# cloudflare/zkp-ecdsa

Hardware: AMD Instinct MI355X
Metric: proveSignatureList proofs/sec (higher is better)
Workload: dtype u32 (9x30-bit limbs, 256/258-bit modular integers); 1 GPU; B=65536 proofs/GPU/step, ring=65536 keys (n=16), per-key tables, secLevel=80, P-256+Tom-256, 24-bit combs, chunk=22016 x 3 lanes; parallelism=single GPU

## Files before the change

zkp-ecdsa_amd/csrc/engine.h:

```cpp
#pragma once
#include <hip/hip_runtime.h>
#include <stdint.h>
#include <atomic>
#include <cstdlib>
#include "../../include/zkattest.h"
#include "curve.h"
#include "rng.h"

struct Soa {
    uint32_t* p;
    uint32_t stride;
};
struct Soa3 {
    Soa x, y, z;
};
template <class M, int K = 2>
ZK_DEV Fe<M, K> soa_ld(const Soa& a, uint32_t e) {
    Fe<M, K> r;
#pragma unroll
    for (int l = 0; l < NLIMB; l++) r.l[l] = a.p[(size_t)l * a.stride + e];
    return r;
}
template <class M, int K>
ZK_DEV void soa_st(const Soa& a, uint32_t e, const Fe<M, K>& v) {
// ... 174 lines not shown
    uint32_t* t1_cnt;
    uint8_t* vbytes;
    uint32_t* vc;
    uint8_t* ph_msg;
    uint32_t* ph_wk;
    uint8_t* ph_nblk;
    TomList vd;
    Soa gk_f, gk_g;
    uint32_t* gk_swap;
    Soa gk_total;
    uint32_t* gk_csub;
    VTerms slot_terms, gk_terms, misc_terms;
    uint8_t* slot_class;
    uint32_t* slot_perm;
    uint32_t* slot_cnt;
    Soa4 slot_acc, gk_acc, misc_acc;
    Soa4 wide_acc;
    Soa sSg, sSh, sSkx, sSky, sSR, sSH, sSL;
    Soa pSR, pSH, pSL;
    Soa pa_x, pa_y, pa_sc;
    uint32_t* pa_tab;
    uint8_t* pa_dig;
    Soa3 pacc;
    Soa clx, cly;
    uint32_t* cl_tab;
    uint8_t* cl_dig;
    uint32_t* p256_ok;
};
void launch_offsets_monotonic(hipStream_t s, const uint64_t* d_off, uint64_t B, uint32_t* d_bad );
void launch_v_unpack(hipStream_t s, uint32_t sec, uint32_t count, const uint8_t* packed, const uint64_t* poff, uint64_t first, uint64_t base, uint8_t* out, uint64_t* uoff);
void launch_v_header_validate(hipStream_t s, const VWork& V, uint32_t count, const uint8_t* proofs, const uint64_t* off, uint64_t first);
void launch_v_front_r(hipStream_t s, const Workspace& W, const VWork& V, uint32_t count, const uint8_t* proofs, const uint64_t* off, uint64_t first);
void launch_v_front_q(hipStream_t s, const DevParams& P, const Workspace& W, const VWork& V, uint32_t count, const uint8_t* proofs, const uint64_t* off, const uint8_t* msg, uint64_t first);
void launch_v_challenges(hipStream_t s, const VWork& V, uint32_t count, const uint8_t* proofs, const uint64_t* off, const uint8_t* msg, uint64_t first, uint32_t parts);
void launch_v_exp_challenge_small(hipStream_t s, const Workspace& W, const VWork& V, uint32_t count, const uint8_t* proofs, const uint64_t* off, uint64_t first);
void launch_v_sample(hipStream_t s, const VWork& V, uint32_t count, const uint8_t* vseeds, uint64_t first);
void launch_v_sample_check(hipStream_t s, const VWork& V, uint32_t count);
void launch_v_exp_status(hipStream_t s, const Workspace& W, const VWork& V, uint32_t count, bool have_jm);
#define V_PH_MAXP 64
#define V_PH_BLOCKS 10
void launch_sha_msgs(hipStream_t s, const Workspace& W, uint32_t count, uint32_t* chal, uint32_t nblk, uint32_t ostride, const uint8_t* nblk_of = nullptr);
void launch_exph_hash(hipStream_t s, const Workspace& W, uint32_t count, uint32_t* chal);
void launch_v_exp_points(hipStream_t s, const Workspace& W, const VWork& V, uint32_t count, const uint8_t* proofs, const uint64_t* off, uint64_t first, uint32_t split = 1);
void launch_v_t1_scalars(hipStream_t s, const Workspace& W, const VWork& V, uint32_t count, const uint8_t* proofs, const uint64_t* off, uint64_t first);
void launch_v_derived(hipStream_t s, const Workspace& W, const VWork& V, uint32_t count, const uint8_t* proofs, const uint64_t* off, uint64_t first);
void launch_v_padd_hash(hipStream_t s, const DevParams& P, const Workspace& W, const VWork& V, uint32_t count, const uint8_t* proofs, const uint64_t* off, uint64_t first);
void launch_v_gk_total(hipStream_t s, const VWork& V, const Soa& ring, const uint32_t* etab, const int8_t* kdig, uint32_t count, uint32_t N, const uint8_t* proofs, const uint64_t* off, uint64_t first, const Soa& res, const Soa& res2);
#define GKM_MINN 12
size_t gkm_ring_frag_bytes(uint64_t N);
size_t gkm_coef_frag_bytes(uint32_t C);
void launch_gkm_ring_digits(hipStream_t s, const Soa& ring, uint32_t nblocks, int8_t* frag);
void launch_gkm_ring_digits_list(hipStream_t s, const Soa& ring, const uint32_t* d_blocks, uint32_t nb, int8_t* frag);
void launch_v_gk_block_mfma(hipStream_t s, const VWork& V, const int8_t* ring_frag, uint32_t nblocks, uint32_t count, int8_t* coef_frag, const Soa& res);
struct ChunkIn;
size_t gkm_etab_frag_bytes(uint64_t N);
size_t gkm_asub_frag_bytes(uint32_t C);
void launch_gkm_etab_digits(hipStream_t s, const uint32_t* E, uint32_t nblocks, int8_t* edig);
void launch_gkm_etab_digits_list(hipStream_t s, const uint32_t* E, uint32_t nblocks, const uint32_t* d_blocks, uint32_t nb, int8_t* edig);
void launch_gk_block_mfma(hipStream_t s, const Workspace& W, const ChunkIn& in, uint32_t nblocks, const Soa& res);
void launch_v_slot_points(hipStream_t s, const VWork& V, uint32_t count, const uint8_t* proofs, const uint64_t* off, uint64_t first);
void launch_v_slot_terms(hipStream_t s, const Workspace& W, const VWork& V, uint32_t count, const uint8_t* proofs, const uint64_t* off, const uint8_t* vseeds, uint64_t first);
void launch_v_proof_points(hipStream_t s, const VWork& V, uint32_t count, const uint8_t* proofs, const uint64_t* off, uint64_t first, uint32_t which);
void launch_v_proof_terms(hipStream_t s, const Workspace& W, const VWork& V, uint32_t count, const uint8_t* proofs, const uint64_t* off, const uint8_t* vseeds, uint64_t first);
void launch_v_proof_sums(hipStream_t s, const Workspace& W, const VWork& V, uint32_t count);
void launch_v_straus(hipStream_t s, const VTerms& L, uint32_t ngroups, uint32_t ng_stride, uint32_t n256, uint32_t n128, const Soa4& out,
                     const uint32_t* perm, const uint32_t* cnt, uint32_t tsplit = 1, uint32_t ostride = 1, uint32_t ny = 1, uint32_t ystride = 0);
void launch_v_acc_tree(hipStream_t s, const Soa4& src, uint32_t nouter, uint32_t width, const Soa4& dst, uint32_t dstride, uint32_t fill);
#ifndef ZK_COOP_MAX_CHAINS
#define ZK_COOP_MAX_CHAINS 16384u
#endif
#ifndef ZK_SCREEN_CO_MAX
#define ZK_SCREEN_CO_MAX 4096u
#endif
extern std::atomic<uint64_t> g_coop_chains;
static inline bool zk_one_lane_chains() {
    static const bool v = getenv("ZKATTEST_ONE_LANE_CHAINS") != nullptr;
    return v;
}
void launch_v_straus_co(hipStream_t s, const VTerms& L, uint32_t ngroups, uint32_t ng_stride, uint32_t n256, uint32_t n128, const Soa4& out, const uint32_t* perm,
                        const uint32_t* cnt, uint32_t tsplit, uint32_t ostride, uint32_t ny, uint32_t ystride);
void launch_v_p256_straus_co(hipStream_t s, const VWork& V, uint32_t count);
void launch_v_exp_points_co(hipStream_t s, const Workspace& W, const VWork& V, uint32_t count, const uint8_t* proofs, const uint64_t* off, uint64_t first);
void launch_rtab_base_co(hipStream_t s, const Workspace& W, uint32_t count, uint32_t bits, const uint8_t* skip);
void launch_v_slot_perm(hipStream_t s, const uint8_t* slot_class, uint32_t nslots, uint32_t* perm, uint32_t* cnt);
void launch_v_p256_straus(hipStream_t s, const VWork& V, uint32_t count, uint32_t per);
void launch_v_p256_total(hipStream_t s, const DevParams& P, const Workspace& W, const VWork& V, uint32_t count, uint32_t per);
void launch_v_p256_total_fixed(hipStream_t s, const DevParams& P, const Workspace& W, const VWork& V, uint32_t count);
void launch_v_p256_total_sum(hipStream_t s, const DevParams& P, const Workspace& W, const VWork& V, uint32_t count);
void launch_v_final(hipStream_t s, const Workspace& W, const VWork& V, uint32_t count, uint8_t* ok, int32_t* status, uint64_t first, const VGroupFlags& gf, uint32_t gsz);
void launch_v_final_memb(hipStream_t s, const Workspace& W, const VWork& V, uint32_t count, uint8_t* ok, int32_t* status, uint64_t first);
void launch_lv_census(hipStream_t s, uint64_t B, const uint8_t* proofs, const uint64_t* off, bool packed, uint8_t* cls, uint32_t* blk_cnt, uint32_t* out);
void launch_lv_perm(hipStream_t s, uint64_t B, const uint8_t* cls, const uint32_t* blk_base, const uint32_t* out, uint32_t* perm);
void launch_lv_gather_meta(hipStream_t s, uint32_t n, const uint32_t* sel, const uint64_t* off, const uint8_t* msg, const uint8_t* vseeds, uint64_t* w_off, uint8_t* w_msg,
                           uint8_t* w_seeds);
void launch_lv_gather_bytes(hipStream_t s, uint32_t n, const uint32_t* sel, const uint64_t* off, const uint8_t* proofs, const uint64_t* w_off, uint8_t* w_bytes);
void launch_lv_scatter(hipStream_t s, uint32_t n, const uint32_t* sel, const uint8_t* w_ok, const int32_t* w_st, uint8_t* ok, int32_t* status, int32_t st);
#define LV_BLOCK 1024
#define RG_UNKNOWN (ZK_MAX_RINGS * ZK_LV_CLASSES)
#define RG_CLASSES (RG_UNKNOWN + 1)
struct RingSlots {
    uint32_t id[ZK_MAX_RINGS];
    uint32_t count;
};
void launch_rg_census(hipStream_t s, uint64_t B, const uint32_t* ring_ids, const RingSlots& rs, const uint8_t* proofs, const uint64_t* off, bool packed, bool per_proof,
                      uint16_t* cls, uint32_t* blk_cnt, uint32_t* out);
void launch_rg_perm(hipStream_t s, uint64_t B, const uint16_t* cls, const uint32_t* blk_base, const uint32_t* out, uint32_t* perm);
// ... 334 lines not shown
```

zkp-ecdsa_amd/csrc/k_gk.hip:

```cpp
#include "engine.h"

#define GKB_BITS 8
#define GKB_SIZE 256

struct GkRankTab {
    uint8_t subset[256];
    uint8_t rank[256];
    uint16_t kstart[10];
};
constexpr GkRankTab gk_make_rank_tab() {
    GkRankTab t{};
    int r = 0;
    for (int k = 0; k <= 8; k++) {
        t.kstart[k] = (uint16_t)r;
        for (int s = 0; s < 256; s++) {
            int pc = 0;
            for (int b = 0; b < 8; b++) pc += (s >> b) & 1;
            if (pc == 8 - k) t.subset[r] = (uint8_t)s, t.rank[s] = (uint8_t)r, r++;
        }
    }
    t.kstart[9] = (uint16_t)r;
    return t;
}
__device__ const GkRankTab GK_RT = gk_make_rank_tab();

__global__ void __launch_bounds__(256) k_gk_etab(Soa ring, uint32_t nblocks, const uint32_t* __restrict__ blist, uint32_t nb, uint32_t* E) {
    uint64_t t = (uint64_t)blockIdx.x * blockDim.x + threadIdx.x;
    uint64_t total = (uint64_t)GKB_SIZE * GKB_SIZE * nb;
    if (t >= total) return;
    uint32_t block = (uint32_t)(t % nb);
    if (blist) block = blist[block];
    uint32_t lr = (uint32_t)(t / nb);
    uint32_t rank = lr & 255, llow = lr >> 8;
    uint32_t S = GK_RT.subset[rank];
    uint32_t fixed = llow & ~S;
    uint32_t pcS = __popc(S);
    Fe<ModQ, 1> acc = fe_zero<ModQ>();
    for (uint32_t T = S;; T = (T - 1) & S) {
        Fe<ModQ, 1> v = soa_ld<ModQ, 1>(ring, block * GKB_SIZE + (fixed | T));
        bool neg = (pcS - __popc(T)) & 1;
        acc = neg ? fe_sub_mod(acc, v) : fe_add_mod(acc, v);
        if (T == 0) break;
    }
    uint32_t o[9];
    limbs_repack<30, 29, 9, 9>(o, acc.l);
#pragma unroll
    for (int l = 0; l < 9; l++) E[((size_t)lr * 9 + l) * nblocks + block] = o[l];
}
void launch_gk_etab_list(hipStream_t s, const Soa& ring, uint32_t nblocks, const uint32_t* d_blocks, uint32_t nb, uint32_t* E) {
    uint64_t total = (uint64_t)GKB_SIZE * GKB_SIZE * nb;
    if (!total) return;
    hipLaunchKernelGGL(k_gk_etab, dim3((uint32_t)((total + 255) / 256)), dim3(256), 0, s, ring, nblocks, d_blocks, nb, E);
}
void launch_gk_etab(hipStream_t s, const Soa& ring, uint32_t nblocks, uint32_t* E) { launch_gk_etab_list(s, ring, nblocks, nullptr, nblocks, E); }
size_t gk_etab_words(uint64_t N) { return (size_t)GKB_SIZE * GKB_SIZE * 9 * (N / GKB_SIZE); }

// ... 39 lines not shown
ZK_DEV void gkc_zero(GkCols& a) {
#pragma unroll
    for (int i = 0; i < 18; i++) a.c[i] = 0;
}
ZK_DEV void gkc_carry(GkCols& a) {
#pragma unroll
    for (int i = 0; i < 17; i++) {
        a.c[i + 1] += a.c[i] >> 29;
        a.c[i] &= (1u << 29) - 1;
    }
}
ZK_DEV void gkc_mac(GkCols& a, const uint32_t x[9], const uint32_t y[9]) {
#pragma unroll
    for (int i = 0; i < 9; i++)
#pragma unroll
        for (int j = 0; j < 9; j++) a.c[i + j] = mad64(x[i], y[j], a.c[i + j]);
}
template <bool UNI>
__global__ void __launch_bounds__(256) k_gk_block(Workspace W, ChunkIn in, const uint32_t* __restrict__ E, const uint32_t* __restrict__ asub,
                                                  const uint32_t* __restrict__ order, const uint32_t* __restrict__ goff, uint32_t nblocks, uint32_t nwg, Soa res,
                                                  uint32_t kmask) {
    uint32_t w = blockIdx.x, seg = (nwg + 7) / 8;
    uint32_t widx = (w & 7) * seg + (w >> 3);
    if (widx >= nwg) return;
    uint32_t p, block;
    if (UNI) {
        uint32_t nbg = nblocks >> 8;
        uint32_t lo = 0, hi = GKB_SIZE;
        while (hi - lo > 1) {
            uint32_t mid = (lo + hi) >> 1;
            if (goff[mid] * nbg <= widx) lo = mid;
            else hi = mid;
        }
        uint32_t g0 = goff[lo], cnt = goff[lo + 1] - g0;
        uint32_t r = widx - g0 * nbg;
        p = order[g0 + r % cnt];
        block = (r / cnt) * 256 + threadIdx.x;
    } else {
        uint32_t slot = widx * 256 + threadIdx.x;
        if (slot >= in.count * nblocks) return;
        p = order[slot / nblocks];
        block = slot % nblocks;
    }
    uint32_t which = in.which[p];
    uint32_t llow = which & 255;
    const uint32_t* a = asub + (size_t)p * GKB_SIZE * 9;
    const uint32_t* e = E + (size_t)llow * GKB_SIZE * 9 * nblocks + block;
#pragma unroll 1
    for (uint32_t k = 0; k < 8; k++) {
        if (!((kmask >> k) & 1)) continue;
        GkCols acc;
        gkc_zero(acc);
        uint32_t r0 = GK_RT.kstart[k], r1 = GK_RT.kstart[k + 1];
#pragma unroll 1
        for (uint32_t rb = r0; rb < r1; rb += 7) {
            uint32_t re = rb + 7 < r1 ? rb + 7 : r1;
#pragma unroll 1
            for (uint32_t r = rb; r < re; r++) {
                uint32_t x[9], y[9];
#pragma unroll
                for (int l = 0; l < 9; l++) x[l] = a[r * 9 + l], y[l] = e[((size_t)r * 9 + l) * nblocks];
                gkc_mac(acc, x, y);
            }
            gkc_carry(acc);
        }
        uint32_t t29[18], t30[18];
#pragma unroll
        for (int i = 0; i < 18; i++) t29[i] = (uint32_t)acc.c[i];
        limbs_repack<29, 30, 18, 18>(t30, t29);
        Fe<ModQ, 1> c = fe_canon(redc_wide(t30));
        soa_st(res, (k * W.C + p) * nblocks + block, c);
    }
    soa_st(res, (8 * W.C + p) * nblocks + block, soa_ld<ModQ, 1>(W.ring, block * GKB_SIZE + llow));
}
void launch_gk_block_stage(hipStream_t s, const Workspace& W, const ChunkIn& in, const Soa& am, const Soa& res) {
    uint32_t nblocks = W.N >> GKB_BITS;
    const bool mm = W.gk_edig != nullptr && W.n >= GKM_MINN;
    hipLaunchKernelGGL(k_gk_sort, dim3(1), dim3(320), 0, s, in, W.gk_order, W.gk_goff, mm ? W.gk_toff : nullptr);
    hipLaunchKernelGGL(k_gk_asub, dim3(in.count), dim3(256), 0, s, W, in.count, am, W.gk_asub);
    bool uni = (nblocks & 255) == 0;
    uint32_t nwg = uni ? in.count * (nblocks >> 8) : (uint32_t)(((uint64_t)in.count * nblocks + 255) / 256);
    uint32_t grid = ((nwg + 7) / 8) * 8;
    const uint32_t kmask = mm ? 0x83u : 0xffu;
    if (uni) hipLaunchKernelGGL(k_gk_block<true>, dim3(grid), dim3(256), 0, s, W, in, W.gk_etab, W.gk_asub, W.gk_order, W.gk_goff, nblocks, nwg, res, kmask);
    else hipLaunchKernelGGL(k_gk_block<false>, dim3(grid), dim3(256), 0, s, W, in, W.gk_etab, W.gk_asub, W.gk_order, W.gk_goff, nblocks, nwg, res, kmask);
    if (mm) launch_gk_block_mfma(s, W, in, nblocks, res);
}

__global__ void __launch_bounds__(256) k_v_gk_csub(VWork V, uint32_t count, uint32_t* csub) {
    uint32_t t = gtid();
    if (t >= count * GKB_SIZE) return;
    uint32_t p = t >> 8, i = t & 255;
    Fe<ModQ, 2> acc = fe_one_mont<ModQ>().as<2>();
    bool zero = false;
    for (uint32_t j = 0; j < GKB_BITS; j++) {
        bool swap = V.gk_swap[j * V.C + p] != 0, set = (i >> j) & 1;
        if (swap) zero = zero || !set;
        else if (set) acc = acc * soa_ld<ModQ, 2>(V.gk_f, j * V.C + p);
    }
    Fe<ModQ, 1> c = zero ? fe_zero<ModQ>() : fe_canon(acc);
    uint32_t o[9];
    limbs_repack<30, 29, 9, 9>(o, c.l);
#pragma unroll
    for (int l = 0; l < 9; l++) csub[(size_t)t * 9 + l] = o[l];
}
template <bool UNI>
__global__ void __launch_bounds__(256) k_v_gk_block(uint32_t count, const uint32_t* __restrict__ E, const uint32_t* __restrict__ csub, uint32_t nblocks, Soa res) {
    uint32_t p, block;
    if (UNI) {
        uint32_t nbg = nblocks >> 8;
        p = blockIdx.x / nbg;
        block = (blockIdx.x % nbg) * 256 + threadIdx.x;
    } else {
        uint32_t slot = blockIdx.x * 256 + threadIdx.x;
        if (slot >= count * nblocks) return;
        p = slot / nblocks, block = slot % nblocks;
    }
    const uint32_t* a = csub + (size_t)p * GKB_SIZE * 9;
    const uint32_t* e = E + ((size_t)255 * 9) * nblocks + block;
    const size_t slice = (size_t)GKB_SIZE * 9 * nblocks;
    GkCols acc;
    gkc_zero(acc);
#pragma unroll 1
    for (uint32_t ib = 0; ib < GKB_SIZE; ib += 7) {
        uint32_t ie = ib + 7 < GKB_SIZE ? ib + 7 : GKB_SIZE;
#pragma unroll 1
        for (uint32_t i = ib; i < ie; i++) {
            uint32_t x[9], y[9];
#pragma unroll
            for (int l = 0; l < 9; l++) x[l] = a[i * 9 + l], y[l] = e[i * slice + (size_t)l * nblocks];
            gkc_mac(acc, x, y);
        }
        gkc_carry(acc);
    }
    uint32_t t29[18], t30[18];
#pragma unroll
    for (int i = 0; i < 18; i++) t29[i] = (uint32_t)acc.c[i];
    limbs_repack<29, 30, 18, 18>(t30, t29);
    soa_st(res, p * nblocks + block, fe_canon(redc_wide(t30)));
// ... 7 lines not shown
```

zkp-ecdsa_amd/csrc/k_gk_mfma.hip:

```cpp
#include "engine.h"

typedef int v4i __attribute__((ext_vector_type(4)));
#define GKM_ND 33
#define GKM_NDIAG (2 * GKM_ND - 2)
#define GKM_FRAG 1024
#define GKM_TILE_BYTES (4 * GKM_ND * GKM_FRAG)

ZK_DEV void gkm_digits(const uint32_t w[8], int8_t d[GKM_ND]) {
    uint32_t carry = 0;
#pragma unroll
    for (int u = 0; u < 32; u++) {
        uint32_t t = ((w[u >> 2] >> (8 * (u & 3))) & 255u) + carry;
        carry = t >= 128u;
        d[u] = (int8_t)(carry ? (int)t - 256 : (int)t);
    }
    d[32] = (int8_t)carry;
}
ZK_DEV size_t gkm_addr(uint32_t tile, uint32_t r, uint32_t i, uint32_t u) {
    const uint32_t kc = i >> 6, g = (i >> 4) & 3, j = i & 15;
    return ((size_t)(tile * 4 + kc) * GKM_ND + u) * GKM_FRAG + (size_t)((g << 4) | r) * 16 + j;
}
__global__ void __launch_bounds__(256) k_gkm_ring_digits(Soa ring, const uint32_t* __restrict__ blist, uint32_t nb, int8_t* frag) {
    uint32_t t = gtid();
    if (t >= nb * 256) return;
    uint32_t block = blist ? blist[t >> 8] : t >> 8, i = t & 255;
    uint32_t w[8];
    words_from_limbs<8>(w, soa_ld<ModQ, 1>(ring, block * 256 + i).l);
    int8_t d[GKM_ND];
    gkm_digits(w, d);
#pragma unroll
    for (int u = 0; u < GKM_ND; u++) frag[gkm_addr(block >> 4, block & 15, i, u)] = d[u];
}
__global__ void __launch_bounds__(256) k_gkm_coef_digits(VWork V, uint32_t count, int8_t* frag) {
    uint32_t t = gtid();
    if (t >= count * 256) return;
    uint32_t p = t >> 8, i = t & 255;
    Fe<ModQ, 2> acc = fe_one_mont<ModQ>().as<2>();
    bool zero = false;
    for (uint32_t j = 0; j < 8; j++) {
        bool swap = V.gk_swap[j * V.C + p] != 0, set = (i >> j) & 1;
        if (swap) zero = zero || !set;
        else if (set) acc = acc * soa_ld<ModQ, 2>(V.gk_f, j * V.C + p);
    }
    Fe<ModQ, 1> c = zero ? fe_zero<ModQ>() : fe_canon(acc);
    uint32_t w[8];
    words_from_limbs<8>(w, c.l);
    int8_t d[GKM_ND];
    gkm_digits(w, d);
#pragma unroll
    for (int u = 0; u < GKM_ND; u++) frag[gkm_addr(p >> 4, p & 15, i, u)] = d[u];
}

ZK_DEV v4i gkm_ld(const int8_t* base, uint32_t lane) { return *(const v4i*)(base + (size_t)lane * 16); }

ZK_DEV void gkm_mfma_row(int u, const v4i& a, const v4i (&b)[GKM_ND], v4i (&acc)[GKM_NDIAG]) {
#pragma unroll
    for (int v = 0; v < GKM_ND; v++) {
        if (u + v < GKM_NDIAG) acc[u + v] = __builtin_amdgcn_mfma_i32_16x16x64_i8(a, b[v], acc[u + v], 0, 0, 0);
        else acc[GKM_NDIAG - 1] = __builtin_amdgcn_mfma_i32_16x16x64_i8(a << 4, b[v] << 4, acc[GKM_NDIAG - 1], 0, 0, 0);
    }
}
template <int V0, int NV>
ZK_DEV void gkm_mfma_row_part(int u, const v4i& a, const v4i (&b)[NV], v4i (&acc)[GKM_NDIAG]) {
#pragma unroll
    for (int v = V0; v < V0 + NV; v++) {
        if (u + v < GKM_NDIAG) acc[u + v] = __builtin_amdgcn_mfma_i32_16x16x64_i8(a, b[v - V0], acc[u + v], 0, 0, 0);
        else acc[GKM_NDIAG - 1] = __builtin_amdgcn_mfma_i32_16x16x64_i8(a << 4, b[v - V0] << 4, acc[GKM_NDIAG - 1], 0, 0, 0);
    }
}
#ifndef GKM_DOUBLE_BUFFER
#define GKM_DOUBLE_BUFFER 0
#endif
#define GKM_H0 17
#define GKM_H1 (GKM_ND - GKM_H0)
ZK_DEV void gkm_chunk_halves(const int8_t* ak, const int8_t* bnext, uint32_t lane, v4i (&b0)[GKM_H0], v4i (&b1)[GKM_H1], v4i (&acc)[GKM_NDIAG]) {
    {
        v4i a0 = gkm_ld(ak, lane), a1 = gkm_ld(ak + GKM_FRAG, lane), a2;
#pragma unroll
        for (int u = 0; u < GKM_ND; u++) {
            if (u + 2 < GKM_ND) a2 = gkm_ld(ak + (size_t)(u + 2) * GKM_FRAG, lane);
            gkm_mfma_row_part<0, GKM_H0>(u, a0, b0, acc);
            a0 = a1, a1 = a2;
        }
    }
    if (bnext) {
#pragma unroll
        for (int v = 0; v < GKM_H0; v++) b0[v] = gkm_ld(bnext + (size_t)v * GKM_FRAG, lane);
    }
    {
        v4i a0 = gkm_ld(ak, lane), a1 = gkm_ld(ak + GKM_FRAG, lane), a2;
#pragma unroll
        for (int u = 0; u < GKM_ND; u++) {
            if (u + 2 < GKM_ND) a2 = gkm_ld(ak + (size_t)(u + 2) * GKM_FRAG, lane);
            gkm_mfma_row_part<GKM_H0, GKM_H1>(u, a0, b1, acc);
            a0 = a1, a1 = a2;
        }
    }
    if (bnext) {
#pragma unroll
        for (int v = 0; v < GKM_H1; v++) b1[v] = gkm_ld(bnext + (size_t)(GKM_H0 + v) * GKM_FRAG, lane);
    }
}

ZK_DEV void gkm_recombine(const int32_t D[GKM_NDIAG], uint32_t t30[18]) {
    uint8_t by[72];
    int64_t c = 0;
#pragma unroll
    for (int d = 0; d < GKM_NDIAG; d++) {
        c += D[d];
        by[d] = (uint8_t)(c & 255);
        c >>= 8;
    }
#pragma unroll
    for (int d = GKM_NDIAG; d < 72; d++) {
        by[d] = (uint8_t)(c & 255);
        c >>= 8;
    }
#pragma unroll
    for (int k = 0; k < 18; k++) {
        const int bit = 30 * k, b0 = bit >> 3, sh = bit & 7;
        uint64_t v = 0;
#pragma unroll
        for (int q = 0; q < 5; q++)
            if (b0 + q < 72) v |= (uint64_t)by[b0 + q] << (8 * q);
        t30[k] = (uint32_t)(v >> sh) & LIMB_MASK;
    }
}

template <int NJ>
ZK_DEV void gkm_recombine_n(const int32_t (&D)[NJ][GKM_NDIAG], uint32_t (&t30)[NJ][18]) {
    int64_t c[NJ] = {};
    uint64_t buf[NJ] = {};
    int nb = 0, k = 0;
#pragma unroll
    for (int d = 0; d < 72; d++) {
#pragma unroll
        for (int j = 0; j < NJ; j++) {
            if (d < GKM_NDIAG) c[j] += D[j][d];
            buf[j] |= (uint64_t)(c[j] & 255) << nb;
            c[j] >>= 8;
        }
        nb += 8;
        if (nb >= 30 && k < 18) {
#pragma unroll
            for (int j = 0; j < NJ; j++) t30[j][k] = (uint32_t)buf[j] & LIMB_MASK, buf[j] >>= 30;
            k++, nb -= 30;
        }
    }
#pragma unroll
    for (int kk = 0; kk < 18; kk++)
        if (kk >= k) {
#pragma unroll
            for (int j = 0; j < NJ; j++) t30[j][kk] = (uint32_t)buf[j] & LIMB_MASK, buf[j] >>= 30;
        }
}
template <int NJ>
ZK_DEV void redc_wide_n(const uint32_t (&T)[NJ][18], Fe<ModQ, 2> (&r)[NJ]) {
    uint64_t a[NJ] = {};
    uint32_t m[NJ][NLIMB];
#pragma unroll
    for (int k = 0; k < NLIMB; k++) {
#pragma unroll
        for (int j = 0; j < NJ; j++) a[j] += T[j][k];
#pragma unroll
        for (int i = 0; i < k; i++)
#pragma unroll
            for (int j = 0; j < NJ; j++) a[j] = mad64(m[j][i], ModQ::mod[k - i], a[j]);
#pragma unroll
        for (int j = 0; j < NJ; j++) {
            m[j][k] = ((uint32_t)a[j] * ModQ::n0) & LIMB_MASK;
            a[j] = mad64(m[j][k], ModQ::mod[0], a[j]);
            a[j] >>= LIMB_BITS;
        }
    }
#pragma unroll
    for (int k = NLIMB; k < 2 * NLIMB; k++) {
#pragma unroll
        for (int j = 0; j < NJ; j++) a[j] += T[j][k];
#pragma unroll
        for (int i = k - (NLIMB - 1); i < NLIMB; i++)
#pragma unroll
            for (int j = 0; j < NJ; j++) a[j] = mad64(m[j][i], ModQ::mod[k - i], a[j]);
#pragma unroll
        for (int j = 0; j < NJ; j++) {
            if (k < 2 * NLIMB - 1) r[j].l[k - NLIMB] = (uint32_t)a[j] & LIMB_MASK, a[j] >>= LIMB_BITS;
            else r[j].l[NLIMB - 1] = (uint32_t)a[j];
        }
    }
}
__global__ void __launch_bounds__(256, 1) k_v_gk_block_mfma(uint32_t count, const int8_t* __restrict__ afrag, const int8_t* __restrict__ bfrag, uint32_t nblocks, uint32_t nkc, Soa res) {
    const uint32_t lane = threadIdx.x & 63, wave = threadIdx.x >> 6;
    const uint32_t tiles_p = (count + 15) >> 4, tiles_b = nblocks >> 4;
    const uint32_t g = blockIdx.x, xcd = g & 7, slot = g >> 3;
    const uint32_t rects_b = (tiles_b + 7) >> 3;
    const uint32_t rect = (slot >> 5) * 8 + xcd, in = slot & 31;
    const uint32_t rp = rect / rects_b, rb = rect % rects_b;
    const uint32_t tile_p = rp * 16 + (in & 15), tile_b = rb * 8 + (in >> 4) * 4 + wave;
    if (tile_p >= tiles_p || tile_b >= tiles_b) return;
    v4i acc[GKM_NDIAG];
#pragma unroll
    for (int d = 0; d < GKM_NDIAG; d++) acc[d] = (v4i){0, 0, 0, 0};
    const int8_t* ap = afrag + (size_t)tile_p * GKM_TILE_BYTES;
    const int8_t* bp = bfrag + (size_t)tile_b * GKM_TILE_BYTES;
#if GKM_DOUBLE_BUFFER
    {
        v4i b0[GKM_H0], b1[GKM_H1];
#pragma unroll
        for (int v = 0; v < GKM_H0; v++) b0[v] = gkm_ld(bp + (size_t)v * GKM_FRAG, lane);
#pragma unroll
        for (int v = 0; v < GKM_H1; v++) b1[v] = gkm_ld(bp + (size_t)(GKM_H0 + v) * GKM_FRAG, lane);
#pragma unroll 1
        for (uint32_t kc = 0; kc < nkc; kc++)
            gkm_chunk_halves(ap + (size_t)kc * GKM_ND * GKM_FRAG, kc + 1 < nkc ? bp + (size_t)(kc + 1) * GKM_ND * GKM_FRAG : nullptr, lane, b0, b1, acc);
    }
#else
#pragma unroll 1
    for (uint32_t kc = 0; kc < nkc; kc++) {
        const int8_t* ak = ap + (size_t)kc * GKM_ND * GKM_FRAG;
        const int8_t* bk = bp + (size_t)kc * GKM_ND * GKM_FRAG;
        v4i b[GKM_ND];
#pragma unroll
        for (int v = 0; v < GKM_ND; v++) b[v] = gkm_ld(bk + (size_t)v * GKM_FRAG, lane);
        v4i a0 = gkm_ld(ak, lane), a1 = gkm_ld(ak + GKM_FRAG, lane), a2;
#pragma unroll
        for (int u = 0; u < GKM_ND; u++) {
            if (u + 2 < GKM_ND) a2 = gkm_ld(ak + (size_t)(u + 2) * GKM_FRAG, lane);
            gkm_mfma_row(u, a0, b, acc);
            a0 = a1, a1 = a2;
        }
    }
#endif
    const uint32_t pb = tile_p * 16 + 4 * (lane >> 4), block = tile_b * 16 + (lane & 15);
#pragma unroll 1
    for (int h = 0; h < 2; h++) {
        int32_t D[2][GKM_NDIAG];
#pragma unroll
        for (int d = 0; d < GKM_NDIAG; d++) D[0][d] = h ? acc[d].z : acc[d].x, D[1][d] = h ? acc[d].w : acc[d].y;
        uint32_t t30[2][18];
        gkm_recombine_n<2>(D, t30);
        Fe<ModQ, 2> r2[2];
        redc_wide_n<2>(t30, r2);
#pragma unroll
        for (int j = 0; j < 2; j++)
            if (pb + 2 * h + j < count) soa_st(res, (pb + 2 * h + j) * nblocks + block, fe_canon(r2[j]));
    }
}

size_t gkm_ring_frag_bytes(uint64_t N) { return (size_t)(N >> 12) * GKM_TILE_BYTES; }
size_t gkm_coef_frag_bytes(uint32_t C) { return (size_t)((C + 15) >> 4) * GKM_TILE_BYTES; }
void launch_gkm_ring_digits_list(hipStream_t s, const Soa& ring, const uint32_t* d_blocks, uint32_t nb, int8_t* frag) {
    if (nb) hipLaunchKernelGGL(k_gkm_ring_digits, dim3(nb), dim3(256), 0, s, ring, d_blocks, nb, frag);
}
void launch_gkm_ring_digits(hipStream_t s, const Soa& ring, uint32_t nblocks, int8_t* frag) { launch_gkm_ring_digits_list(s, ring, nullptr, nblocks, frag); }
void launch_v_gk_block_mfma(hipStream_t s, const VWork& V, const int8_t* ring_frag, uint32_t nblocks, uint32_t count, int8_t* coef_frag, const Soa& res) {
    hipLaunchKernelGGL(k_gkm_coef_digits, dim3(count), dim3(256), 0, s, V, count, coef_frag);
    const uint32_t tiles_p = (count + 15) >> 4, tiles_b = nblocks >> 4;
    const uint32_t rects = ((tiles_p + 15) >> 4) * ((tiles_b + 7) >> 3);
    const uint32_t nwg = ((rects + 7) / 8) * 8 * 32;
    hipLaunchKernelGGL(k_v_gk_block_mfma, dim3(nwg), dim3(256), 0, s, count, coef_frag, ring_frag, nblocks, 4u, res);
}

#define GKP_CHUNKS 6
__device__ const uint8_t GKP_BASE[GKP_CHUNKS] = {9, 37, 93, 157, 163, 219};
__device__ const uint8_t GKP_CNT[GKP_CHUNKS] = {28, 56, 64, 6, 56, 28};
#define GKP_TILE_BYTES (GKP_CHUNKS * GKM_ND * GKM_FRAG)
ZK_DEV void gkp_place(uint32_t rank, uint32_t& c, uint32_t& kpos) {
    c = rank < 37 ? 0 : rank < 93 ? 1 : rank < 157 ? 2 : rank < 163 ? 3 : rank < 219 ? 4 : 5;
    kpos = rank - GKP_BASE[c];
}
ZK_DEV size_t gkp_addr(size_t tile, uint32_t r, uint32_t c, uint32_t kpos, uint32_t u) {
    return ((tile * GKP_CHUNKS + c) * GKM_ND + u) * GKM_FRAG + (size_t)((((kpos >> 4) & 3) << 4) | r) * 16 + (kpos & 15);
}
__global__ void __launch_bounds__(256) k_gkm_etab_digits(const uint32_t* __restrict__ E, uint32_t nblocks, const uint32_t* __restrict__ blist, uint32_t nb, int8_t* edig) {
    uint64_t t = (uint64_t)blockIdx.x * blockDim.x + threadIdx.x;
    uint64_t total = (uint64_t)256 * 238 * nb;
    if (t >= total) return;
    uint32_t block = (uint32_t)(t % nb);
    if (blist) block = blist[block];
    uint32_t lr = (uint32_t)(t / nb), rank = 9 + lr % 238, llow = lr / 238;
    uint32_t l29[9], l30[9], w[8];
#pragma unroll
    for (int l = 0; l < 9; l++) l29[l] = E[(((size_t)llow * 256 + rank) * 9 + l) * nblocks + block];
    limbs_repack<29, 30, 9, 9>(l30, l29);
    words_from_limbs<8>(w, l30);
    int8_t d[GKM_ND];
    gkm_digits(w, d);
    uint32_t c, kpos;
    gkp_place(rank, c, kpos);
    const size_t tile = (size_t)llow * (nblocks >> 4) + (block >> 4);
#pragma unroll
    for (int u = 0; u < GKM_ND; u++) edig[gkp_addr(tile, block & 15, c, kpos, u)] = d[u];
}
__global__ void __launch_bounds__(256) k_gkm_asub_digits(ChunkIn in, const uint32_t* __restrict__ asub, const uint32_t* __restrict__ order, const uint32_t* __restrict__ goff,
                                                         const uint32_t* __restrict__ toff, int8_t* adig) {
    uint32_t t = gtid();
    if (t >= in.count * 238) return;
    uint32_t pos = t / 238, rank = 9 + t % 238;
    uint32_t p = order[pos], g = in.which[p] & 255, idx = pos - goff[g];
    uint32_t l29[9], l30[9], w[8];
#pragma unroll
    for (int l = 0; l < 9; l++) l29[l] = asub[((size_t)p * 256 + rank) * 9 + l];
    limbs_repack<29, 30, 9, 9>(l30, l29);
    words_from_limbs<8>(w, l30);
    int8_t d[GKM_ND];
    gkm_digits(w, d);
    uint32_t c, kpos;
    gkp_place(rank, c, kpos);
    const size_t tile = toff[g] + (idx >> 4);
#pragma unroll
    for (int u = 0; u < GKM_ND; u++) adig[gkp_addr(tile, idx & 15, c, kpos, u)] = d[u];
}
__global__ void __launch_bounds__(256, 1) k_gk_block_mfma(Workspace W, ChunkIn in, const int8_t* __restrict__ adig, const int8_t* __restrict__ edig,
                                                         const uint32_t* __restrict__ order, const uint32_t* __restrict__ goff, const uint32_t* __restrict__ toff,
                                                         uint32_t nblocks, uint32_t tiles_max, Soa res) {
    const uint32_t lane = threadIdx.x & 63, wave = threadIdx.x >> 6;
    const uint32_t tiles_b = nblocks >> 4, wgb = (tiles_b + 3) >> 2;
    const uint32_t nwork = tiles_max * wgb, seg = (nwork + 7) >> 3;
    const uint32_t widx = (blockIdx.x & 7) * seg + (blockIdx.x >> 3);
    if (widx >= nwork || (blockIdx.x >> 3) >= seg) return;
    const uint32_t t = widx % tiles_max, tile_b = (widx / tiles_max) * 4 + wave;
    if (t >= toff[256] || tile_b >= tiles_b) return;
    uint32_t lo = 0, hi = 256;
    while (hi - lo > 1) {
        uint32_t mid = (lo + hi) >> 1;
        if (toff[mid] <= t) lo = mid;
        else hi = mid;
    }
    const uint32_t g = lo, g0 = goff[g], gcnt = goff[g + 1] - g0, row0 = (t - toff[g]) * 16;
    const int8_t* ap = adig + (size_t)t * GKP_TILE_BYTES;
    const int8_t* bp = edig + ((size_t)g * tiles_b + tile_b) * GKP_TILE_BYTES;
    const uint32_t cls = blockIdx.y, c0 = cls < 3 ? cls : cls + 1, c1 = cls == 2 ? 4 : c0 + 1, k = cls + 2;
    v4i acc[GKM_NDIAG];
#pragma unroll
    for (int d = 0; d < GKM_NDIAG; d++) acc[d] = (v4i){0, 0, 0, 0};
#if GKM_DOUBLE_BUFFER
    {
        const int8_t* bk0 = bp + (size_t)c0 * GKM_ND * GKM_FRAG;
        v4i b0[GKM_H0], b1[GKM_H1];
#pragma unroll
        for (int v = 0; v < GKM_H0; v++) b0[v] = gkm_ld(bk0 + (size_t)v * GKM_FRAG, lane);
#pragma unroll
        for (int v = 0; v < GKM_H1; v++) b1[v] = gkm_ld(bk0 + (size_t)(GKM_H0 + v) * GKM_FRAG, lane);
#pragma unroll 1
        for (uint32_t c = c0; c < c1; c++)
            gkm_chunk_halves(ap + (size_t)c * GKM_ND * GKM_FRAG, c + 1 < c1 ? bp + (size_t)(c + 1) * GKM_ND * GKM_FRAG : nullptr, lane, b0, b1, acc);
    }
#else
#pragma unroll 1
    for (uint32_t c = c0; c < c1; c++) {
        const int8_t* ak = ap + (size_t)c * GKM_ND * GKM_FRAG;
        const int8_t* bk = bp + (size_t)c * GKM_ND * GKM_FRAG;
        v4i b[GKM_ND];
#pragma unroll
        for (int v = 0; v < GKM_ND; v++) b[v] = gkm_ld(bk + (size_t)v * GKM_FRAG, lane);
        v4i a0 = gkm_ld(ak, lane), a1 = gkm_ld(ak + GKM_FRAG, lane), a2;
#pragma unroll
        for (int u = 0; u < GKM_ND; u++) {
            if (u + 2 < GKM_ND) a2 = gkm_ld(ak + (size_t)(u + 2) * GKM_FRAG, lane);
            gkm_mfma_row(u, a0, b, acc);
            a0 = a1, a1 = a2;
        }
    }
#endif
    const uint32_t rowb = row0 + 4 * (lane >> 4), block = tile_b * 16 + (lane & 15);
#pragma unroll 1
    for (int h = 0; h < 2; h++) {
        int32_t D[2][GKM_NDIAG];
#pragma unroll
        for (int d = 0; d < GKM_NDIAG; d++) D[0][d] = h ? acc[d].z : acc[d].x, D[1][d] = h ? acc[d].w : acc[d].y;
        uint32_t t30[2][18];
        gkm_recombine_n<2>(D, t30);
        Fe<ModQ, 2> r2[2];
        redc_wide_n<2>(t30, r2);
#pragma unroll
        for (int j = 0; j < 2; j++) {
            const uint32_t row = rowb + 2 * h + j;
            if (row < gcnt) soa_st(res, (k * W.C + order[g0 + row]) * nblocks + block, fe_canon(r2[j]));
        }
    }
}
size_t gkm_etab_frag_bytes(uint64_t N) { return (size_t)256 * (N >> 12) * GKP_TILE_BYTES; }
size_t gkm_asub_frag_bytes(uint32_t C) { return (size_t)((C >> 4) + 256 + 1) * GKP_TILE_BYTES; }
void launch_gkm_etab_digits(hipStream_t s, const uint32_t* E, uint32_t nblocks, int8_t* edig) {
    hipMemsetAsync(edig, 0, gkm_etab_frag_bytes((uint64_t)nblocks << 8), s);
    uint64_t total = (uint64_t)256 * 238 * nblocks;
    hipLaunchKernelGGL(k_gkm_etab_digits, dim3((uint32_t)((total + 255) / 256)), dim3(256), 0, s, E, nblocks, nullptr, nblocks, edig);
}
__global__ void __launch_bounds__(256) k_gkm_etab_clear(uint32_t nblocks, const uint32_t* __restrict__ blist, uint32_t nb, int8_t* edig) {
    uint64_t t = (uint64_t)blockIdx.x * blockDim.x + threadIdx.x;
    uint64_t total = (uint64_t)256 * GKP_CHUNKS * GKM_ND * 4 * nb;
    if (t >= total) return;
    const uint32_t block = blist[(uint32_t)(t % nb)];
    uint32_t q = (uint32_t)(t / nb);
    const uint32_t g = q & 3;
    q >>= 2;
    const uint32_t u = q % GKM_ND, c = (q / GKM_ND) % GKP_CHUNKS, llow = q / (GKM_ND * GKP_CHUNKS);
    const size_t tile = (size_t)llow * (nblocks >> 4) + (block >> 4);
    *(uint4*)(edig + gkp_addr(tile, block & 15, c, g << 4, u)) = make_uint4(0, 0, 0, 0);
}
void launch_gkm_etab_digits_list(hipStream_t s, const uint32_t* E, uint32_t nblocks, const uint32_t* d_blocks, uint32_t nb, int8_t* edig) {
    if (!nb) return;
    uint64_t total = (uint64_t)256 * GKP_CHUNKS * GKM_ND * 4 * nb;
    hipLaunchKernelGGL(k_gkm_etab_clear, dim3((uint32_t)((total + 255) / 256)), dim3(256), 0, s, nblocks, d_blocks, nb, edig);
    total = (uint64_t)256 * 238 * nb;
    hipLaunchKernelGGL(k_gkm_etab_digits, dim3((uint32_t)((total + 255) / 256)), dim3(256), 0, s, E, nblocks, d_blocks, nb, edig);
}
void launch_gk_block_mfma(hipStream_t s, const Workspace& W, const ChunkIn& in, uint32_t nblocks, const Soa& res) {
    const uint32_t tiles_max = (in.count >> 4) + 256;
    hipMemsetAsync(W.gk_adig, 0, (size_t)tiles_max * GKP_TILE_BYTES, s);
    hipLaunchKernelGGL(k_gkm_asub_digits, dim3((in.count * 238 + 255) / 256), dim3(256), 0, s, in, W.gk_asub, W.gk_order, W.gk_goff, W.gk_toff, W.gk_adig);
    const uint32_t wgb = ((nblocks >> 4) + 3) >> 2;
    hipLaunchKernelGGL(k_gk_block_mfma, dim3(((tiles_max * wgb + 7) >> 3) << 3, 5), dim3(256), 0, s, W, in, W.gk_adig, W.gk_edig, W.gk_order, W.gk_goff, W.gk_toff, nblocks, tiles_max, res);
}
```

Baseline: 361,000 proofs/s.

## Pack narrow GK MFMA chunks, move k=4 tail ranks to scalar kernel

Reworks the int8 MFMA fragment layout for the per-key GK block products. The two 28-rank chunks now use half-width (8-byte) fragments instead of padding to 64, cutting fragment storage, loads and zero-padded MFMA work. The six tail ranks (157..163) are dropped from the MFMA path and handled by the scalar k_gk_block kernel, which adds them to the MFMA result. To make that accumulation valid, the MFMA launch now runs before the scalar kernel. The unused double-buffer path is removed. The cost is extra scalar work and a read-modify-write of the k=4 results, plus a more intricate addressing scheme.

```diff
diff --git a/zkp-ecdsa_amd/csrc/engine.h b/zkp-ecdsa_amd/csrc/engine.h
--- a/zkp-ecdsa_amd/csrc/engine.h
+++ b/zkp-ecdsa_amd/csrc/engine.h
@@ -250,6 +250,8 @@
 void launch_gkm_ring_digits(hipStream_t s, const Soa& ring, uint32_t nblocks, int8_t* frag);
 void launch_gkm_ring_digits_list(hipStream_t s, const Soa& ring, const uint32_t* d_blocks, uint32_t nb, int8_t* frag);
 void launch_v_gk_block_mfma(hipStream_t s, const VWork& V, const int8_t* ring_frag, uint32_t nblocks, uint32_t count, int8_t* coef_frag, const Soa& res);
+#define GKP_TAIL0 157
+#define GKP_TAIL1 163
 struct ChunkIn;
 size_t gkm_etab_frag_bytes(uint64_t N);
 size_t gkm_asub_frag_bytes(uint32_t C);
diff --git a/zkp-ecdsa_amd/csrc/k_gk.hip b/zkp-ecdsa_amd/csrc/k_gk.hip
--- a/zkp-ecdsa_amd/csrc/k_gk.hip
+++ b/zkp-ecdsa_amd/csrc/k_gk.hip
@@ -2,6 +2,7 @@
 
 #define GKB_BITS 8
 #define GKB_SIZE 256
+#define GK_KMASK_TAIL4 0x100u
 
 struct GkRankTab {
     uint8_t subset[256];
@@ -147,6 +148,8 @@
         GkCols acc;
         gkc_zero(acc);
         uint32_t r0 = GK_RT.kstart[k], r1 = GK_RT.kstart[k + 1];
+        const bool tail = k == 4 && (kmask & GK_KMASK_TAIL4);
+        if (tail) r0 = GKP_TAIL0, r1 = GKP_TAIL1;
 #pragma unroll 1
         for (uint32_t rb = r0; rb < r1; rb += 7) {
             uint32_t re = rb + 7 < r1 ? rb + 7 : r1;
@@ -164,6 +167,7 @@
         for (int i = 0; i < 18; i++) t29[i] = (uint32_t)acc.c[i];
         limbs_repack<29, 30, 18, 18>(t30, t29);
         Fe<ModQ, 1> c = fe_canon(redc_wide(t30));
+        if (tail) c = fe_add_mod(c, soa_ld<ModQ, 1>(res, (k * W.C + p) * nblocks + block));
         soa_st(res, (k * W.C + p) * nblocks + block, c);
     }
     soa_st(res, (8 * W.C + p) * nblocks + block, soa_ld<ModQ, 1>(W.ring, block * GKB_SIZE + llow));
@@ -176,10 +180,10 @@
     bool uni = (nblocks & 255) == 0;
     uint32_t nwg = uni ? in.count * (nblocks >> 8) : (uint32_t)(((uint64_t)in.count * nblocks + 255) / 256);
     uint32_t grid = ((nwg + 7) / 8) * 8;
-    const uint32_t kmask = mm ? 0x83u : 0xffu;
+    const uint32_t kmask = mm ? 0x93u | GK_KMASK_TAIL4 : 0xffu;
+    if (mm) launch_gk_block_mfma(s, W, in, nblocks, res);
     if (uni) hipLaunchKernelGGL(k_gk_block<true>, dim3(grid), dim3(256), 0, s, W, in, W.gk_etab, W.gk_asub, W.gk_order, W.gk_goff, nblocks, nwg, res, kmask);
     else hipLaunchKernelGGL(k_gk_block<false>, dim3(grid), dim3(256), 0, s, W, in, W.gk_etab, W.gk_asub, W.gk_order, W.gk_goff, nblocks, nwg, res, kmask);
-    if (mm) launch_gk_block_mfma(s, W, in, nblocks, res);
 }
 
 __global__ void __launch_bounds__(256) k_v_gk_csub(VWork V, uint32_t count, uint32_t* csub) {
diff --git a/zkp-ecdsa_amd/csrc/k_gk_mfma.hip b/zkp-ecdsa_amd/csrc/k_gk_mfma.hip
--- a/zkp-ecdsa_amd/csrc/k_gk_mfma.hip
+++ b/zkp-ecdsa_amd/csrc/k_gk_mfma.hip
@@ -60,48 +60,6 @@
         else acc[GKM_NDIAG - 1] = __builtin_amdgcn_mfma_i32_16x16x64_i8(a << 4, b[v] << 4, acc[GKM_NDIAG - 1], 0, 0, 0);
     }
 }
-template <int V0, int NV>
-ZK_DEV void gkm_mfma_row_part(int u, const v4i& a, const v4i (&b)[NV], v4i (&acc)[GKM_NDIAG]) {
-#pragma unroll
-    for (int v = V0; v < V0 + NV; v++) {
-        if (u + v < GKM_NDIAG) acc[u + v] = __builtin_amdgcn_mfma_i32_16x16x64_i8(a, b[v - V0], acc[u + v], 0, 0, 0);
-        else acc[GKM_NDIAG - 1] = __builtin_amdgcn_mfma_i32_16x16x64_i8(a << 4, b[v - V0] << 4, acc[GKM_NDIAG - 1], 0, 0, 0);
-    }
-}
-#ifndef GKM_DOUBLE_BUFFER
-#define GKM_DOUBLE_BUFFER 0
-#endif
-#define GKM_H0 17
-#define GKM_H1 (GKM_ND - GKM_H0)
-ZK_DEV void gkm_chunk_halves(const int8_t* ak, const int8_t* bnext, uint32_t lane, v4i (&b0)[GKM_H0], v4i (&b1)[GKM_H1], v4i (&acc)[GKM_NDIAG]) {
-    {
-        v4i a0 = gkm_ld(ak, lane), a1 = gkm_ld(ak + GKM_FRAG, lane), a2;
-#pragma unroll
-        for (int u = 0; u < GKM_ND; u++) {
-            if (u + 2 < GKM_ND) a2 = gkm_ld(ak + (size_t)(u + 2) * GKM_FRAG, lane);
-            gkm_mfma_row_part<0, GKM_H0>(u, a0, b0, acc);
-            a0 = a1, a1 = a2;
-        }
-    }
-    if (bnext) {
-#pragma unroll
-        for (int v = 0; v < GKM_H0; v++) b0[v] = gkm_ld(bnext + (size_t)v * GKM_FRAG, lane);
-    }
-    {
-        v4i a0 = gkm_ld(ak, lane), a1 = gkm_ld(ak + GKM_FRAG, lane), a2;
-#pragma unroll
-        for (int u = 0; u < GKM_ND; u++) {
-            if (u + 2 < GKM_ND) a2 = gkm_ld(ak + (size_t)(u + 2) * GKM_FRAG, lane);
-            gkm_mfma_row_part<GKM_H0, GKM_H1>(u, a0, b1, acc);
-            a0 = a1, a1 = a2;
-        }
-    }
-    if (bnext) {
-#pragma unroll
-        for (int v = 0; v < GKM_H1; v++) b1[v] = gkm_ld(bnext + (size_t)(GKM_H0 + v) * GKM_FRAG, lane);
-    }
-}
-
 ZK_DEV void gkm_recombine(const int32_t D[GKM_NDIAG], uint32_t t30[18]) {
     uint8_t by[72];
     int64_t c = 0;
@@ -202,18 +160,6 @@
     for (int d = 0; d < GKM_NDIAG; d++) acc[d] = (v4i){0, 0, 0, 0};
     const int8_t* ap = afrag + (size_t)tile_p * GKM_TILE_BYTES;
     const int8_t* bp = bfrag + (size_t)tile_b * GKM_TILE_BYTES;
-#if GKM_DOUBLE_BUFFER
-    {
-        v4i b0[GKM_H0], b1[GKM_H1];
-#pragma unroll
-        for (int v = 0; v < GKM_H0; v++) b0[v] = gkm_ld(bp + (size_t)v * GKM_FRAG, lane);
-#pragma unroll
-        for (int v = 0; v < GKM_H1; v++) b1[v] = gkm_ld(bp + (size_t)(GKM_H0 + v) * GKM_FRAG, lane);
-#pragma unroll 1
-        for (uint32_t kc = 0; kc < nkc; kc++)
-            gkm_chunk_halves(ap + (size_t)kc * GKM_ND * GKM_FRAG, kc + 1 < nkc ? bp + (size_t)(kc + 1) * GKM_ND * GKM_FRAG : nullptr, lane, b0, b1, acc);
-    }
-#else
 #pragma unroll 1
     for (uint32_t kc = 0; kc < nkc; kc++) {
         const int8_t* ak = ap + (size_t)kc * GKM_ND * GKM_FRAG;
@@ -229,7 +175,6 @@
             a0 = a1, a1 = a2;
         }
     }
-#endif
     const uint32_t pb = tile_p * 16 + 4 * (lane >> 4), block = tile_b * 16 + (lane & 15);
 #pragma unroll 1
     for (int h = 0; h < 2; h++) {
@@ -260,24 +205,29 @@
     hipLaunchKernelGGL(k_v_gk_block_mfma, dim3(nwg), dim3(256), 0, s, count, coef_frag, ring_frag, nblocks, 4u, res);
 }
 
-#define GKP_CHUNKS 6
-__device__ const uint8_t GKP_BASE[GKP_CHUNKS] = {9, 37, 93, 157, 163, 219};
-__device__ const uint8_t GKP_CNT[GKP_CHUNKS] = {28, 56, 64, 6, 56, 28};
-#define GKP_TILE_BYTES (GKP_CHUNKS * GKM_ND * GKM_FRAG)
-ZK_DEV void gkp_place(uint32_t rank, uint32_t& c, uint32_t& kpos) {
-    c = rank < 37 ? 0 : rank < 93 ? 1 : rank < 157 ? 2 : rank < 163 ? 3 : rank < 219 ? 4 : 5;
-    kpos = rank - GKP_BASE[c];
-}
-ZK_DEV size_t gkp_addr(size_t tile, uint32_t r, uint32_t c, uint32_t kpos, uint32_t u) {
-    return ((tile * GKP_CHUNKS + c) * GKM_ND + u) * GKM_FRAG + (size_t)((((kpos >> 4) & 3) << 4) | r) * 16 + (kpos & 15);
+#define GKP_CHUNKS 5
+ZK_HD constexpr uint32_t gkp_off(uint32_t c) { return c ? 2 * c - 1 : 0; }
+#define GKP_NARROW(c) ((c) == 0 || (c) == 4)
+#define GKP_FRAG_N (GKM_FRAG / 2)
+#define GKP_TILE_BYTES (8 * GKM_ND * GKP_FRAG_N)
+#define GKP_RANKS (238 - (GKP_TAIL1 - GKP_TAIL0))
+ZK_HD uint32_t gkp_rank(uint32_t i) { return 9 + i + (i >= GKP_TAIL0 - 9 ? GKP_TAIL1 - GKP_TAIL0 : 0); }
+ZK_HD void gkp_place(uint32_t rank, uint32_t& c, uint32_t& kpos) {
+    constexpr uint8_t base[GKP_CHUNKS] = {9, 37, 93, 163, 219};
+    c = rank < 37 ? 0 : rank < 93 ? 1 : rank < 163 ? 2 : rank < 219 ? 3 : 4;
+    kpos = rank - base[c];
+}
+ZK_HD size_t gkp_addr(size_t tile, uint32_t r, uint32_t c, uint32_t kpos, uint32_t u) {
+    const uint32_t sh = GKP_NARROW(c) ? 3 : 4, w = 1u << sh;
+    return tile * GKP_TILE_BYTES + ((size_t)gkp_off(c) * GKM_ND + (size_t)u * (w >> 3)) * GKP_FRAG_N + (size_t)(((kpos >> sh) << 4) | r) * w + (kpos & (w - 1));
 }
 __global__ void __launch_bounds__(256) k_gkm_etab_digits(const uint32_t* __restrict__ E, uint32_t nblocks, const uint32_t* __restrict__ blist, uint32_t nb, int8_t* edig) {
     uint64_t t = (uint64_t)blockIdx.x * blockDim.x + threadIdx.x;
-    uint64_t total = (uint64_t)256 * 238 * nb;
+    uint64_t total = (uint64_t)256 * GKP_RANKS * nb;
     if (t >= total) return;
     uint32_t block = (uint32_t)(t % nb);
     if (blist) block = blist[block];
-    uint32_t lr = (uint32_t)(t / nb), rank = 9 + lr % 238, llow = lr / 238;
+    uint32_t lr = (uint32_t)(t / nb), rank = gkp_rank(lr % GKP_RANKS), llow = lr / GKP_RANKS;
     uint32_t l29[9], l30[9], w[8];
 #pragma unroll
     for (int l = 0; l < 9; l++) l29[l] = E[(((size_t)llow * 256 + rank) * 9 + l) * nblocks + block];
@@ -294,8 +244,8 @@
 __global__ void __launch_bounds__(256) k_gkm_asub_digits(ChunkIn in, const uint32_t* __restrict__ asub, const uint32_t* __restrict__ order, const uint32_t* __restrict__ goff,
                                                          const uint32_t* __restrict__ toff, int8_t* adig) {
     uint32_t t = gtid();
-    if (t >= in.count * 238) return;
-    uint32_t pos = t / 238, rank = 9 + t % 238;
+    if (t >= in.count * GKP_RANKS) return;
+    uint32_t pos = t / GKP_RANKS, rank = gkp_rank(t % GKP_RANKS);
     uint32_t p = order[pos], g = in.which[p] & 255, idx = pos - goff[g];
     uint32_t l29[9], l30[9], w[8];
 #pragma unroll
@@ -309,6 +259,11 @@
     const size_t tile = toff[g] + (idx >> 4);
 #pragma unroll
     for (int u = 0; u < GKM_ND; u++) adig[gkp_addr(tile, idx & 15, c, kpos, u)] = d[u];
+}
+typedef int v2i __attribute__((ext_vector_type(2)));
+ZK_DEV v4i gkp_ld8(const int8_t* base, uint32_t lane) {
+    const v2i lo = *(const v2i*)(base + (size_t)lane * 8);
+    return (v4i){lo.x, lo.y, 0, 0};
 }
 __global__ void __launch_bounds__(256, 1) k_gk_block_mfma(Workspace W, ChunkIn in, const int8_t* __restrict__ adig, const int8_t* __restrict__ edig,
                                                          const uint32_t* __restrict__ order, const uint32_t* __restrict__ goff, const uint32_t* __restrict__ toff,
@@ -327,29 +282,25 @@
         else hi = mid;
     }
     const uint32_t g = lo, g0 = goff[g], gcnt = goff[g + 1] - g0, row0 = (t - toff[g]) * 16;
-    const int8_t* ap = adig + (size_t)t * GKP_TILE_BYTES;
-    const int8_t* bp = edig + ((size_t)g * tiles_b + tile_b) * GKP_TILE_BYTES;
-    const uint32_t cls = blockIdx.y, c0 = cls < 3 ? cls : cls + 1, c1 = cls == 2 ? 4 : c0 + 1, k = cls + 2;
+    const uint32_t c = blockIdx.y, k = c + 2;
+    const size_t coff = (size_t)gkp_off(c) * GKM_ND * GKP_FRAG_N;
+    const int8_t* ak = adig + (size_t)t * GKP_TILE_BYTES + coff;
+    const int8_t* bk = edig + ((size_t)g * tiles_b + tile_b) * GKP_TILE_BYTES + coff;
     v4i acc[GKM_NDIAG];
 #pragma unroll
     for (int d = 0; d < GKM_NDIAG; d++) acc[d] = (v4i){0, 0, 0, 0};
-#if GKM_DOUBLE_BUFFER
-    {
-        const int8_t* bk0 = bp + (size_t)c0 * GKM_ND * GKM_FRAG;
-        v4i b0[GKM_H0], b1[GKM_H1];
-#pragma unroll
-        for (int v = 0; v < GKM_H0; v++) b0[v] = gkm_ld(bk0 + (size_t)v * GKM_FRAG, lane);
-#pragma unroll
-        for (int v = 0; v < GKM_H1; v++) b1[v] = gkm_ld(bk0 + (size_t)(GKM_H0 + v) * GKM_FRAG, lane);
-#pragma unroll 1
-        for (uint32_t c = c0; c < c1; c++)
-            gkm_chunk_halves(ap + (size_t)c * GKM_ND * GKM_FRAG, c + 1 < c1 ? bp + (size_t)(c + 1) * GKM_ND * GKM_FRAG : nullptr, lane, b0, b1, acc);
-    }
-#else
-#pragma unroll 1
-    for (uint32_t c = c0; c < c1; c++) {
-        const int8_t* ak = ap + (size_t)c * GKM_ND * GKM_FRAG;
-        const int8_t* bk = bp + (size_t)c * GKM_ND * GKM_FRAG;
+    if (GKP_NARROW(c)) {
+        v4i b[GKM_ND];
+#pragma unroll
+        for (int v = 0; v < GKM_ND; v++) b[v] = gkp_ld8(bk + (size_t)v * GKP_FRAG_N, lane);
+        v4i a0 = gkp_ld8(ak, lane), a1 = gkp_ld8(ak + GKP_FRAG_N, lane), a2;
+#pragma unroll
+        for (int u = 0; u < GKM_ND; u++) {
+            if (u + 2 < GKM_ND) a2 = gkp_ld8(ak + (size_t)(u + 2) * GKP_FRAG_N, lane);
+            gkm_mfma_row(u, a0, b, acc);
+            a0 = a1, a1 = a2;
+        }
+    } else {
         v4i b[GKM_ND];
 #pragma unroll
         for (int v = 0; v < GKM_ND; v++) b[v] = gkm_ld(bk + (size_t)v * GKM_FRAG, lane);
@@ -361,7 +312,6 @@
             a0 = a1, a1 = a2;
         }
     }
-#endif
     const uint32_t rowb = row0 + 4 * (lane >> 4), block = tile_b * 16 + (lane & 15);
 #pragma unroll 1
     for (int h = 0; h < 2; h++) {
@@ -383,7 +333,7 @@
 size_t gkm_asub_frag_bytes(uint32_t C) { return (size_t)((C >> 4) + 256 + 1) * GKP_TILE_BYTES; }
 void launch_gkm_etab_digits(hipStream_t s, const uint32_t* E, uint32_t nblocks, int8_t* edig) {
     hipMemsetAsync(edig, 0, gkm_etab_frag_bytes((uint64_t)nblocks << 8), s);
-    uint64_t total = (uint64_t)256 * 238 * nblocks;
+    uint64_t total = (uint64_t)256 * GKP_RANKS * nblocks;
     hipLaunchKernelGGL(k_gkm_etab_digits, dim3((uint32_t)((total + 255) / 256)), dim3(256), 0, s, E, nblocks, nullptr, nblocks, edig);
 }
 __global__ void __launch_bounds__(256) k_gkm_etab_clear(uint32_t nblocks, const uint32_t* __restrict__ blist, uint32_t nb, int8_t* edig) {
@@ -396,19 +346,27 @@
     q >>= 2;
     const uint32_t u = q % GKM_ND, c = (q / GKM_ND) % GKP_CHUNKS, llow = q / (GKM_ND * GKP_CHUNKS);
     const size_t tile = (size_t)llow * (nblocks >> 4) + (block >> 4);
-    *(uint4*)(edig + gkp_addr(tile, block & 15, c, g << 4, u)) = make_uint4(0, 0, 0, 0);
+    if (GKP_NARROW(c)) *(uint2*)(edig + gkp_addr(tile, block & 15, c, g << 3, u)) = make_uint2(0, 0);
+    else *(uint4*)(edig + gkp_addr(tile, block & 15, c, g << 4, u)) = make_uint4(0, 0, 0, 0);
 }
 void launch_gkm_etab_digits_list(hipStream_t s, const uint32_t* E, uint32_t nblocks, const uint32_t* d_blocks, uint32_t nb, int8_t* edig) {
     if (!nb) return;
     uint64_t total = (uint64_t)256 * GKP_CHUNKS * GKM_ND * 4 * nb;
     hipLaunchKernelGGL(k_gkm_etab_clear, dim3((uint32_t)((total + 255) / 256)), dim3(256), 0, s, nblocks, d_blocks, nb, edig);
-    total = (uint64_t)256 * 238 * nb;
+    total = (uint64_t)256 * GKP_RANKS * nb;
     hipLaunchKernelGGL(k_gkm_etab_digits, dim3((uint32_t)((total + 255) / 256)), dim3(256), 0, s, E, nblocks, d_blocks, nb, edig);
 }
 void launch_gk_block_mfma(hipStream_t s, const Workspace& W, const ChunkIn& in, uint32_t nblocks, const Soa& res) {
     const uint32_t tiles_max = (in.count >> 4) + 256;
     hipMemsetAsync(W.gk_adig, 0, (size_t)tiles_max * GKP_TILE_BYTES, s);
-    hipLaunchKernelGGL(k_gkm_asub_digits, dim3((in.count * 238 + 255) / 256), dim3(256), 0, s, in, W.gk_asub, W.gk_order, W.gk_goff, W.gk_toff, W.gk_adig);
+    hipLaunchKernelGGL(k_gkm_asub_digits, dim3((in.count * GKP_RANKS + 255) / 256), dim3(256), 0, s, in, W.gk_asub, W.gk_order, W.gk_goff, W.gk_toff, W.gk_adig);
     const uint32_t wgb = ((nblocks >> 4) + 3) >> 2;
-    hipLaunchKernelGGL(k_gk_block_mfma, dim3(((tiles_max * wgb + 7) >> 3) << 3, 5), dim3(256), 0, s, W, in, W.gk_adig, W.gk_edig, W.gk_order, W.gk_goff, W.gk_toff, nblocks, tiles_max, res);
-}
+    hipLaunchKernelGGL(k_gk_block_mfma, dim3(((tiles_max * wgb + 7) >> 3) << 3, GKP_CHUNKS), dim3(256), 0, s, W, in, W.gk_adig, W.gk_edig, W.gk_order, W.gk_goff, W.gk_toff, nblocks, tiles_max, res);
+}
+extern "C" int zk_test_gkp_place(uint32_t rank, uint32_t r, uint32_t u, uint64_t out[3]) {
+    if (rank < 9 || rank > 246 || (rank >= GKP_TAIL0 && rank < GKP_TAIL1) || r > 15 || u >= GKM_ND) return 0;
+    uint32_t c, kpos;
+    gkp_place(rank, c, kpos);
+    out[0] = c, out[1] = kpos, out[2] = gkp_addr(0, r, c, kpos, u);
+    return 1;
+}
```

After: 359,300 proofs/s. About the same (-0.5%).
